# JasperSnoek/spearmint

Measured on AMD Instinct MI355X. Metric: EI candidate evaluations per second (N_cand x mcmc_iters / wall time), higher is better.
Workload: dtype f64; 1 GPU; C3: synthetic 32D, N_obs=2048, 200k candidates/GPU, mcmc_iters=20; N_obs=2048, candidates_per_gpu=200000, D=32, mcmc_iters=20, collective=torch.distributed all_gather_into_tensor

## Files before the change

### spearmint_amd/csrc/common.h

```cpp
#pragma once
#include <hip/hip_runtime.h>
#include <stdint.h>

typedef double d4 __attribute__((ext_vector_type(4)));
typedef double d2 __attribute__((ext_vector_type(2)));

#define MFMA_F64(a, b, c) __builtin_amdgcn_mfma_f64_16x16x4f64((a), (b), (c), 0, 0, 0)

#define SPX_NB 64
#define SPX_BM 128
#define SPX_BN 128
#define SPX_BK 16
#define SPX_PADN 128

#define SPX_COV_MATERN52 0
#define SPX_COV_MATERN32 1
#define SPX_COV_ARDSE 2

#define SPX_HT 4

static inline int64_t round_up(int64_t x, int64_t m) { return (x + m - 1) / m * m; }

void spx_note_attr_error(const char* kernel, size_t lds_bytes, hipError_t e);
#define SPX_LDS_ATTR(fn, bytes)                                                                                            \
// ... 5 lines not shown

void launch_scale_rows(hipStream_t s, const double* x, int64_t n, int64_t n_pad, int D, int Dp,
                       const double* ls , int ls_stride, int nh, double factor,
                       double* xs , double* sumsq ,
                       double* xs2 = nullptr ,
                       int* zero_ints = nullptr , int n_zero = 0);
void launch_lean_prologue(hipStream_t s, const double* x, int64_t n, int64_t n_pad, int D, int Dp, const double* ls,
                          int ls_stride, int nh, double* xs, double* sumsq, double* xs2, const double* vals,
                          const double* htab, double* rhs, int* info, int* flags, int64_t vals_stride = 0);
void launch_cov_self(hipStream_t s, const double* Xs, const double* s1, const double* X2s,
                     const double* htab, double* K, int N, int Np, int Dp, int nh, bool tiled = false,
                     int kind = SPX_COV_MATERN52);
void launch_cov_cross(hipStream_t s, const double* Xs, const double* s1, const double* Cs,
                      const double* s2, const double* htab, double* Kst, int N, int Np, int Mc,
                      int Dp, int nh, int kind = SPX_COV_MATERN52, int live_rows = 0 ,
                      bool allow_flat = true );
void launch_cross_mean(hipStream_t s, const double* Xs, const double* s1, const double* Cs,
                       const double* s2, const double* htab, const double* alpha, double* out,
                       int N, int Np, int Mc, int Dp, int nh, int kind = SPX_COV_MATERN52);
void launch_constraint_prob(hipStream_t s, const double* Xs, const double* s1, const double* Cs,
                            const double* s2, const double* htab, const double* alpha, double* out,
                            int N, int Np, int Mc, int Dp, int nh, int kind);
void launch_constraint_const(hipStream_t s, const double* htab, double* out, int Mc, int nh);

void launch_chol_diag(hipStream_t s, double* L, double* Dinv, int* info, int Np, int k, int nh, int updated = 0);
void launch_chol_panel(hipStream_t s, double* L, const double* Dinv, int Np, int k, int nh, double* rhs = nullptr);
void launch_lean_step(hipStream_t s, double* Lt, double* Dinv, int* info, double* rhs, double* diagL, int Np, int k,
                      int nh, int lazy);
void launch_lean_trsm(hipStream_t s, double* Lt, const double* Dinv, double* rhs, int Np, int k, int nh);
void launch_lean_step_ps(hipStream_t s, double* Lt, double* Dinv, int* info, double* rhs, double* diagL, int* flags,
                         int Np, int k, int nh);
// ... 55 lines not shown
    double* uvec;
};
void launch_point_finish(hipStream_t s, const FinishArgs& a, bool constrained);

void launch_ei_fused128(hipStream_t s, int kind, const double* WT, const double* gamma, const double* Xs, const double* s1,
                        const double* Cs, const double* s2, const double* htab, const double* time_m, const double* cprob, double best,
                        double* ei_draw, double* mom_m, double* mom_v, int N, int Mc, int Dp, int nh, int64_t c0,
                        int64_t M, int64_t Mp, int n_cu);

void launch_sobol_grid(hipStream_t s, const uint32_t* dirs, int dim, int64_t n, int64_t skip, double* out);

void launch_predict_gemm(hipStream_t s, int variant, const double* WT, const double* Kst, const double* gamma,
                         double* part_ss, double* part_bg, int Np, int Mc, int nh, int part_nh, int part_h0,
                         const double* gammaS = nullptr, int S = 0, double* part_bgS = nullptr, int nlive = 0);
bool predict_gemm_variant_ok(int v);
int predict_gemm_padding_plan(int variant, int N, int Np);
void launch_ei_finalize_fant(hipStream_t s, const double* part_ss, const double* part_bgS,
                             const double* htab, const double* bests, const double* time_m, const double* cprob,
                             double* ei_draw, int nrb, int Mc, int nh, int S, int64_t c0, int64_t M,
                             int64_t Mp, int h0, double* ei_s);
void launch_ei_finalize(hipStream_t s, const double* part_ss, const double* part_bg,
                        const double* htab, const double* time_m, const double* cprob, double best, double* ei_draw,
                        double* mom_m, double* mom_v, int nrb, int Mc, int nh, int64_t c0,
                        int64_t M, int64_t Mp, int h0);
void launch_mean_over_draws(hipStream_t s, const double* ei_draw, double* ei_mean, int64_t M,
                            int64_t Mp, int H);
void launch_sum_over_draws(hipStream_t s, const double* ei_draw, double* out, int64_t M, int64_t Mp, int H);
void launch_div_scalar(hipStream_t s, double* v, int64_t n, double denom);
void launch_argmax(hipStream_t s, const double* v, int64_t M, double* blk_val, int64_t* blk_idx,
                   double* out_val, int64_t* out_idx, double* host_mirror = nullptr, const int* info = nullptr, int n_info = 0);
// ... 5 lines not shown
```

### spearmint_amd/csrc/cov_kernels.hip

```cpp
#include "common.h"
#include "ei_device.h"

#ifndef SPX_COV_HOIST
#define SPX_COV_HOIST 1
#endif

#define SR_DC 32
template <int ROWS>
__device__ __forceinline__ void scale_rows_body(
    const double* __restrict__ x, int64_t n, int64_t n_pad, int D, int Dp,
    const double* __restrict__ ls, int ls_stride, double factor,
    double* __restrict__ xs, double* __restrict__ sumsq, double* __restrict__ xs2, int bx, int h)
{
#pragma clang fp contract(off)
    __shared__ double T[ROWS][SR_DC + 1];
    const int tid = threadIdx.x;
    const int64_t row0 = (int64_t)bx * ROWS;
    const int rows = (int)((n_pad - row0 < ROWS) ? (n_pad - row0) : ROWS);
    const int64_t row = row0 + tid;
    const double* lsh = ls + (size_t)h * ls_stride;
    double* o = xs + ((size_t)h * n_pad + row0) * Dp;
    double* o2 = xs2 ? xs2 + ((size_t)h * n_pad + row0) * Dp : nullptr;
    double acc = 0.0;
    for (int d0 = 0; d0 < Dp; d0 += SR_DC) {
// ... 242 lines not shown

template <int MODE, int QC, int KIND>
__global__ __launch_bounds__(256, 2) void k_cov(
    const double* __restrict__ Xs, const double* __restrict__ s1,
    const double* __restrict__ Cs, const double* __restrict__ s2,
    const double* __restrict__ htab, const double* __restrict__ alpha,
    double* __restrict__ out, int N, int Np, int Mc, int Dp, int nchunks, int64_t ldo, int rows_per_wg, int live_rows)
{
    const int jtop = (MODE == 0 && live_rows > 0) ? live_rows : Np;
    const int jbeg = (MODE == 2 || MODE == 4) ? 0 : blockIdx.y * rows_per_wg;
    const int jend = (MODE == 2 || MODE == 4) ? Np : min(jtop, jbeg + rows_per_wg);
    cov_run<MODE, QC, KIND>(Xs, s1, Cs, s2, htab, alpha, out, N, Np, Mc, Dp, nchunks, ldo, blockIdx.z, blockIdx.x * 64, jbeg, jend);
}

template <int QC, int KIND>
__global__ __launch_bounds__(256, 2) void k_cov_flat(
    const double* __restrict__ Xs, const double* __restrict__ s1,
    const double* __restrict__ Cs, const double* __restrict__ s2,
    const double* __restrict__ htab, double* __restrict__ out, int N, int Np, int Mc, int Dp, int nchunks, int64_t ldo, int nh,
    int live_rows)
{
    const int jtop = live_rows > 0 ? live_rows : Np;
    const int nrc = (jtop + 127) >> 7, ncb = Mc >> 6;
    const int64_t per_h = (int64_t)ncb * nrc, U = per_h * nh;
    int64_t u = U * blockIdx.x / gridDim.x;
    const int64_t u1 = U * (blockIdx.x + 1) / gridDim.x;
    while (u < u1) {
        const int h = (int)(u / per_h);
        const int rem = (int)(u - (int64_t)h * per_h);
        const int cb = rem / nrc, rc = rem - cb * nrc;
        const int run = (int)min((int64_t)(nrc - rc), u1 - u);
        cov_run<0, QC, KIND>(Xs, s1, Cs, s2, htab, nullptr, out, N, Np, Mc, Dp, nchunks, ldo, h, cb * 64, rc * 128,
                             min(jtop, (rc + run) * 128));
        u += run;
    }
}

template <int MODE, int KIND>
static void launch_cov_kind(hipStream_t s, const double* Xs, const double* s1, const double* Cs,
                            const double* s2, const double* htab, const double* alpha, double* out,
                            int N, int Np, int Mc, int Dp, int nh, int64_t ldo, int live_rows, bool allow_flat)
{
    const int Q = Dp / 4;
    int rows_per_wg = (Np >= 1024) ? 512 : ((Np >= 256) ? 256 : 128);
#ifdef SPX_DEV_KNOBS
    static const char* rpw = getenv("SPX_COV_RPW");
    if (rpw && MODE == 3) rows_per_wg = atoi(rpw);
#endif
    const int row_top = (MODE == 0 && live_rows > 0) ? live_rows : Np;
    dim3 grid(Mc / 64, (MODE == 2 || MODE == 4) ? 1 : (row_top + rows_per_wg - 1) / rows_per_wg, nh);
// ... 25 lines not shown
}

template <int MODE>
static void launch_cov_mode(hipStream_t s, int kind, const double* Xs, const double* s1, const double* Cs,
                            const double* s2, const double* htab, const double* alpha, double* out,
                            int N, int Np, int Mc, int Dp, int nh, int64_t ldo, int live_rows = 0, bool allow_flat = true)
{
    if (kind == SPX_COV_MATERN32)
        launch_cov_kind<MODE, SPX_COV_MATERN32>(s, Xs, s1, Cs, s2, htab, alpha, out, N, Np, Mc, Dp, nh, ldo, live_rows, allow_flat);
    else if (kind == SPX_COV_ARDSE)
        launch_cov_kind<MODE, SPX_COV_ARDSE>(s, Xs, s1, Cs, s2, htab, alpha, out, N, Np, Mc, Dp, nh, ldo, live_rows, allow_flat);
    else
        launch_cov_kind<MODE, SPX_COV_MATERN52>(s, Xs, s1, Cs, s2, htab, alpha, out, N, Np, Mc, Dp, nh, ldo, live_rows, allow_flat);
}

void launch_cov_cross(hipStream_t s, const double* Xs, const double* s1, const double* Cs,
                      const double* s2, const double* htab, double* Kst, int N, int Np, int Mc,
                      int Dp, int nh, int kind, int live_rows, bool allow_flat)
{
    launch_cov_mode<0>(s, kind, Xs, s1, Cs, s2, htab, nullptr, Kst, N, Np, Mc, Dp, nh, Mc, live_rows, allow_flat);
}

void launch_cov_self(hipStream_t s, const double* Xs, const double* s1, const double* X2s,
                     const double* htab, double* K, int N, int Np, int Dp, int nh, bool tiled, int kind)
{
    if (tiled) launch_cov_mode<3>(s, kind, Xs, s1, X2s, s1, htab, nullptr, K, N, Np, Np, Dp, nh, Np);
    else launch_cov_mode<1>(s, kind, Xs, s1, X2s, s1, htab, nullptr, K, N, Np, Np, Dp, nh, Np);
}

void launch_cross_mean(hipStream_t s, const double* Xs, const double* s1, const double* Cs,
                       const double* s2, const double* htab, const double* alpha, double* out,
                       int N, int Np, int Mc, int Dp, int nh, int kind)
{
    launch_cov_mode<2>(s, kind, Xs, s1, Cs, s2, htab, alpha, out, N, Np, Mc, Dp, nh, Mc);
// ... 21 lines not shown
```

### spearmint_amd/csrc/predict_kernels.hip

```cpp
#include "common.h"
#include "np_sum.h"
#include "ei_device.h"

#define BM SPX_BM
#define BN SPX_BN
#define BK SPX_BK
#define LDT 144

template <int NW, int STG, int ABL>
__global__ __launch_bounds__(64 * NW, NW / 2) void k_predict_gemm(
    const double* __restrict__ WT, const double* __restrict__ Kst,
    const double* __restrict__ gamma, double* __restrict__ part_ss,
    double* __restrict__ part_bg, int Np, int Mc, int nh, int ncb, int nrb,
    int part_nh , int part_h0 ,
    const double* __restrict__ gammaS , int S,
    double* __restrict__ part_bgS )
{
    extern __shared__ __attribute__((aligned(16))) double smem[];
    double* As = smem;
    double* Bs = smem + 2 * BK * LDT;

    const int tid = threadIdx.x;
    const int lane = tid & 63, wave = tid >> 6;
    const int g = lane >> 4, li = lane & 15;
// ... 204 lines not shown
#pragma unroll
            for (int nt = 0; nt < 4; ++nt) {
                double bg = 0.0;
#pragma unroll
                for (int mt = 0; mt < MT; ++mt)
#pragma unroll
                    for (int r = 0; r < 4; ++r) bg = fma(acc[mt][nt][r], gv[mt][r], bg);
                bg += __shfl_xor(bg, 16);
                bg += __shfl_xor(bg, 32);
                if (g == 0) outS[(size_t)sidx * Mc + 16 * nt + li] = bg;
            }
        }
    }
}

__global__ __launch_bounds__(256, 2) void k_predict_gemm_tri(
    const double* __restrict__ WT, const double* __restrict__ Kst,
    const double* __restrict__ gamma, double* __restrict__ part_ss,
    double* __restrict__ part_bg, int Np, int Mc, int nh, int ncb, int nrb,
    int part_nh, int part_h0, const double* __restrict__ gammaS, int S, double* __restrict__ part_bgS)
{
    extern __shared__ __attribute__((aligned(16))) double smem[];
    double* As = smem;
    double* Bs = smem + 2 * BK * LDT;
    const int tid = threadIdx.x;
    const int lane = tid & 63;
    const int wave = __builtin_amdgcn_readfirstlane(tid >> 6);
    const int g = lane >> 4, li = lane & 15;
    const int wm = wave >> 1, wn = wave & 1;
    constexpr int NW = 4, NQ = 4;

    const int ncbx = (ncb + 7) >> 3;
    const int xcd = blockIdx.x & 7;
    const int slot = blockIdx.x >> 3;
    const int per_rb = ncbx * nh;
    const int ib = nrb - 1 - slot / per_rb;
// ... 39 lines not shown
        if (m0 == 0) {
#pragma unroll
            for (int k0 = 0; k0 < BK; k0 += 4) {
                double a[4], b[4];
#pragma unroll
                for (int t = 0; t < 4; ++t) b[t] = Bc[(k0 + g) * LDT + 16 * t];
#pragma unroll
                for (int t = 0; t < 4; ++t) a[t] = Ac[(k0 + g) * LDT + 32 * t];
#pragma unroll
                for (int mt = 0; mt < 4; ++mt)
#pragma unroll
                    for (int nt = 0; nt < 4; ++nt) acc[mt][nt] = MFMA_F64(a[mt], b[nt], acc[mt][nt]);
            }
            asm volatile("s_waitcnt vmcnt(0)" ::: "memory");
            __syncthreads();
        } else {
#define SPX_TRI_G4(MT_)                                                      \
    _Pragma("unroll") for (int nt = 0; nt < 4; ++nt) acc[MT_][nt] = MFMA_F64(a[MT_], b[nt], acc[MT_][nt]);
#pragma unroll
            for (int k0 = 0; k0 < BK; k0 += 4) {
                double a[4], b[4];
#pragma unroll
                for (int t = 0; t < 4; ++t) b[t] = Bc[(k0 + g) * LDT + 16 * t];
#pragma unroll
                for (int t = 0; t < 4; ++t) a[t] = Ac[(k0 + g) * LDT + 32 * t];
                switch (m0) {
                    case 1: SPX_TRI_G4(1)
                    case 2: SPX_TRI_G4(2)
                    case 3: SPX_TRI_G4(3)
                    default: break;
                }
            }
#undef SPX_TRI_G4
            asm volatile("s_waitcnt vmcnt(0)" ::: "memory");
            __syncthreads();
        }
        cur ^= 1;
    }
#undef SPX_DMA_TILE
#undef SPX_DMA_ROW

    const double* gh = gamma + (size_t)h * Np + (size_t)ib * BM + 16 * wm;
    double gam[4][4];
#pragma unroll
    for (int mt = 0; mt < 4; ++mt)
#pragma unroll
        for (int r = 0; r < 4; ++r) gam[mt][r] = gh[32 * mt + g + 4 * r];
    double* red = smem;
// ... 44 lines not shown
                bg += __shfl_xor(bg, 16);
                bg += __shfl_xor(bg, 32);
                if (g == 0) outS[(size_t)sidx * Mc + 16 * nt + li] = bg;
            }
        }
    }
}

template <int ML>
__global__ __launch_bounds__(256, 2) void k_predict_gemm_tail(
    const double* __restrict__ WT, const double* __restrict__ Kst,
    const double* __restrict__ gamma, double* __restrict__ part_ss,
    double* __restrict__ part_bg, int Np, int Mc, int nh, int ncb, int ib, int nlive,
    int part_nh, int part_h0, const double* __restrict__ gammaS, int S, double* __restrict__ part_bgS)
{
    extern __shared__ __attribute__((aligned(16))) double smem[];
    double* As = smem;
    double* Bs = smem + 2 * BK * LDT;
    const int tid = threadIdx.x;
    const int lane = tid & 63;
    const int wave = __builtin_amdgcn_readfirstlane(tid >> 6);
    const int g = lane >> 4, li = lane & 15;
    const int wm = wave >> 1, wn = wave & 1;
    constexpr int NW = 4, NQ = 4;

    const int ncbx = (ncb + 7) >> 3;
    const int xcd = blockIdx.x & 7;
    const int slot = blockIdx.x >> 3;
    const int h = slot / ncbx;
    const int cb = (slot % ncbx) * 8 + xcd;
// ... 139 lines not shown
        default: return false;
    }
}

template <int NW, int STG, int ABL>
static void launch_gemm_variant(hipStream_t s, int grid, size_t lds, const double* WT, const double* Kst,
                                const double* gamma, double* part_ss, double* part_bg, int Np, int Mc, int nh,
                                int ncb, int nrb, int part_nh, int part_h0, const double* gammaS, int S,
                                double* part_bgS)
{
    SPX_LDS_ATTR((k_predict_gemm<NW, STG, ABL>), lds);
    hipLaunchKernelGGL((k_predict_gemm<NW, STG, ABL>), dim3(grid), dim3(64 * NW), lds, s, WT, Kst, gamma, part_ss,
                       part_bg, Np, Mc, nh, ncb, nrb, part_nh, part_h0, gammaS, S, part_bgS);
}

void launch_predict_gemm(hipStream_t s, int variant, const double* WT, const double* Kst, const double* gamma,
                         double* part_ss, double* part_bg, int Np, int Mc, int nh, int part_nh, int part_h0,
                         const double* gammaS, int S, double* part_bgS, int nlive)
{
    const int ncb = Mc / BN, nrb = Np / BM;
    const size_t lds = (size_t)(4 * BK * LDT) * sizeof(double);
    const int grid = 8 * ((ncb + 7) / 8) * nrb * nh;
#define SPX_GO(NW_, STG_, ABL_)                                                                               \
    launch_gemm_variant<NW_, STG_, ABL_>(s, grid, lds, WT, Kst, gamma, part_ss, part_bg, Np, Mc, nh, ncb, nrb, \
                                         part_nh, part_h0, gammaS, S, part_bgS)
    const int v = (S > 0 && variant != 0 && variant != 32) ? 14 : variant;
    if (v == 0 || v == 32) {
        const bool tail = nlive > 0 && predict_gemm_padding_plan(v, 16 * nlive, Np) == nlive;
        const int nrb_main = tail ? nrb - 1 : nrb;
        if (tail) {
            const int lt = nlive - 8 * (nrb - 1), ml = (lt + 1) / 2;
            const int tgrid = 8 * ((ncb + 7) / 8) * nh;
#define SPX_TAIL(ML_)                                                                                                   \
    do {                                                                                                                \
        SPX_LDS_ATTR(k_predict_gemm_tail<ML_>, lds);                                                                    \
        hipLaunchKernelGGL(k_predict_gemm_tail<ML_>, dim3(tgrid), dim3(256), lds, s, WT, Kst, gamma, part_ss, part_bg, Np, Mc, \
// ... 272 lines not shown
```

### spearmint_amd/csrc/spx_api.hip

```cpp
#include <math.h>
#include <stdarg.h>
#include <stdio.h>
#include <string.h>

#include <algorithm>
#include <string>
#include <vector>

#include <chrono>

#include "spx_internal.h"
#include "np_sum.h"

#define SPX_VERSION 200

static const char* kStageNames[ST_COUNT] = {
    "scale_rows", "cov_self", "chol_diag", "chol_panel", "trinv", "gamma_alpha",
    "cov_cross", "cross_mean", "predict_gemm", "ei_finalize", "mean_argmax",
    "factor_total", "ei_run_total"};


std::string& spx_err_slot()
{
    static thread_local std::string g_err;
// ... 22 lines not shown
    va_start(ap, fmt);
    vsnprintf(buf, sizeof buf, fmt, ap);
    va_end(ap);
    spx_err_slot() = buf;
    if (!spx_attr_err_slot().empty()) {
        spx_err_slot() += " [also: " + spx_attr_err_slot() + "]";
        spx_attr_err_slot().clear();
    }
    return code;
}

static int ensure_init(spx_handle* h)
{
    HIPCHK(hipSetDevice(h->device));
    if (!h->inited) {
        HIPCHK(hipStreamCreateWithFlags(&h->stream, hipStreamNonBlocking));
        HIPCHK(hipStreamCreateWithFlags(&h->stream2, hipStreamNonBlocking));
        for (int i = 0; i < 6; ++i) HIPCHK(hipEventCreateWithFlags(&h->ev_sync[i], hipEventDisableTiming));
        HIPCHK(hipEventCreate(&h->ev_t0));
        HIPCHK(hipEventCreate(&h->ev_t1));
        HIPCHK(hipEventCreateWithFlags(&h->ev_obs, hipEventDisableTiming));
        HIPCHK(hipEventCreateWithFlags(&h->ev_p0, hipEventDisableTiming));
        HIPCHK(hipEventCreateWithFlags(&h->ev_fac, hipEventDisableTiming));
        int ncu = 0;
        if (hipDeviceGetAttribute(&ncu, hipDeviceAttributeMultiprocessorCount, h->device) == hipSuccess && ncu > 0) h->n_cu = ncu;
        h->inited = true;
    }
    return SPX_OK;
}

static int ev_begin(spx_handle* h, int stage, hipStream_t strm)
{
    if (!h->timing) return -1;
    if (h->ev_used == h->ev_pool.size()) {
        spx_handle::Ev e;
        if (hipEventCreate(&e.a) != hipSuccess || hipEventCreate(&e.b) != hipSuccess) return -1;
        h->ev_pool.push_back(e);
    }
    spx_handle::Ev& e = h->ev_pool[h->ev_used];
    e.stage = stage;
    (void)hipEventRecord(e.a, strm);
    return (int)h->ev_used++;
}
static void ev_end(spx_handle* h, int id, hipStream_t strm)
{
// ... 51 lines not shown
    *out = h;
    return SPX_OK;
}

void spx_destroy(spx_handle* h)
{
    if (!h) return;
    if (h->multi) { spx_multi_destroy(h->multi); delete h; return; }
    spx_comm_release(h);
    if (h->con) { spx_destroy(h->con); h->con = nullptr; }
    if (h->full) { spx_destroy(h->full); h->full = nullptr; }
    if (h->inited) {
        (void)hipSetDevice(h->device);
        (void)hipStreamSynchronize(h->stream);
        (void)hipStreamSynchronize(h->stream2);
        DevBuf* bufs[] = {&h->comp, &h->vals, &h->ldur, &h->cand, &h->hyp, &h->htab, &h->Xs, &h->X2s,
                          &h->s1, &h->Lm, &h->WT, &h->Dinv, &h->gamma, &h->alpha, &h->info, &h->lp,
                          &h->Cs[0], &h->s2[0], &h->Kst[0], &h->part_ss[0], &h->part_bg[0], &h->time_m[0],
                          &h->Cs[1], &h->s2[1], &h->Kst[1], &h->part_ss[1], &h->part_bg[1], &h->time_m[1],
                          &h->fantT, &h->gammaS, &h->bests, &h->part_bgS[0], &h->part_bgS[1],
                          &h->pt_x, &h->pt_k, &h->pt_dk, &h->pt_t, &h->pt_z, &h->pt_out, &h->pt_kt, &h->pt_dkt,
                          &h->ei_draw, &h->ei_mean, &h->mom_m, &h->mom_v, &h->mom_t, &h->am_val, &h->am_idx,
                          &h->am_out_val, &h->am_out_idx, &h->scratch, &h->sobol_dirs, &h->sobol_out, &h->rhs, &h->diagL, &h->ps_flags, &h->flow_flags,
                          &h->alphaS, &h->pt_u, &h->rec_send, &h->rec_recv, &h->rec_out, &h->ei_sum_full,
                          &h->con_tab, &h->con_Cs[0], &h->con_Cs[1], &h->con_s2[0], &h->con_s2[1], &h->con_p[0], &h->con_p[1],
                          &h->mom_c, &h->rhs_rows};
        for (DevBuf* b : bufs) b->release();
        h->pin_up.release();
        h->pin_res.release();
        h->pin_stage.release();
// ... 88 lines not shown
    if (!strcmp(name, "lean_poll")) { h->lean_poll = value < 0 ? -1 : (value != 0); return SPX_OK; }
    if (!strcmp(name, "lean_zc")) { h->lean_zc = value < 0 ? -1 : (value != 0); return SPX_OK; }
    if (!strcmp(name, "stage_copies")) {
        h->stage_copies = value < 0 ? -1 : (value != 0);
        return SPX_OK;
    }
    if (!strcmp(name, "cov_flat")) {
        h->cov_flat = value < 0 ? -1 : (value != 0);
        return SPX_OK;
    }
    if (!strcmp(name, "gemm_partial")) {
        h->gemm_partial = value < 0 ? -1 : (value != 0);
        return SPX_OK;
    }
    if (!strcmp(name, "streams")) {
        h->nstreams = value == 2 ? 2 : 1;
        return SPX_OK;
    }
    if (!strcmp(name, "timing")) {
        h->timing = value != 0;
        memset(h->st_ms, 0, sizeof h->st_ms);
        memset(h->st_n, 0, sizeof h->st_n);
        return SPX_OK;
    }
    return fail(SPX_ERR_ARG, "spx_set_option: unknown option '%s'", name);
}

#define SPX_STAGE_MAX (8u << 20)
static void stage_begin(spx_handle* h) { h->stage_off = 0; }
static int stage_h2d(spx_handle* h, void* dst, const void* src, size_t bytes, hipStream_t s)
{
// ... 515 lines not shown
    h->handoff_timeout = false;
    rc = do_factor(h, false, false, true);
    if (rc) return rc;
    h->S = 0;
    rc = ei_run_impl(h, flags, true);
    if (rc == SPX_ERR_HIP && h->handoff_timeout && h->flow_used) {
        note_flow_timeout(h);
        rc = do_factor(h, false);
        if (!rc) rc = ei_run_impl(h, flags, false);
        if (!rc) warn_flow_fallback(h);
        return rc;
    }
    if (rc) {
        (void)hipStreamSynchronize(h->stream);
        (void)hipStreamSynchronize(h->stream2);
        (void)hipGetLastError();
        if (rc != SPX_ERR_NOT_PD) h->factored = false;
    }
    return rc;
}

static int ei_run_impl(spx_handle* h, int32_t flags, bool factor_pending)
{
    if (!h->factored && !factor_pending) return fail(SPX_ERR_ARG, "spx_ei_run: call spx_factor first");
    if (!h->have_cand) return fail(SPX_ERR_ARG, "spx_ei_run: no candidates set");
    const bool per_sec = (flags & SPX_FLAG_PER_SEC) != 0;
    const bool keep_mom = (flags & SPX_FLAG_KEEP_MOMENTS) != 0;
    const bool time_only = (flags & SPX_FLAG_TIME_ONLY) != 0;
    const bool constrained = (flags & SPX_FLAG_CONSTRAINED) != 0;
    int rc = check_run_flags(h, flags, h->nmodels);
// ... 21 lines not shown
        const int64_t fant_budget = h->fant_budget;
        int64_t cap = fant_budget / ((int64_t)nrb * 2 * S * 8) / SPX_BN * SPX_BN;
        if (cap < SPX_BN) cap = SPX_BN;
        if (Mc > cap) {
            const int64_t nchunks = (Mp + cap - 1) / cap;
            Mc = round_up((Mp + nchunks - 1) / nchunks, SPX_BN);
        }
        int64_t hb = fant_budget / ((int64_t)nrb * 2 * S * 8 * Mc);
        if (hb > 65535 / S) hb = 65535 / S;
        if (hb < 1) hb = 1;
        if (hb < Hb) Hb = (int)hb;
    }

    const bool fused = Np == SPX_PADN && S == 0 && h->ei_fused != 0;
    h->last_fused = fused;
    const int ns = fused ? 1 : h->nstreams;
    for (int b = 0; b < 2; ++b) {
        if ((rc = h->Cs[b].reserve((size_t)H * Mc * Dp * 8))) return rc;
        if ((rc = h->s2[b].reserve((size_t)H * Mc * 8))) return rc;
        if (per_sec && (rc = h->time_m[b].reserve((size_t)H * Mc * 8))) return rc;
        if (constrained && (rc = h->con_p[b].reserve((size_t)H * Mc * 8))) return rc;
        if (constrained && h->con_n > 0 && (rc = h->con_Cs[b].reserve((size_t)H * Mc * Dp * 8))) return rc;
        if (constrained && h->con_n > 0 && (rc = h->con_s2[b].reserve((size_t)H * Mc * 8))) return rc;
        if (b < ns && !fused && !time_only) {
            if ((rc = h->Kst[b].reserve((size_t)Hb * Np * Mc * 8))) return rc;
            if (S > 0 && (rc = h->part_bgS[b].reserve((size_t)nrb * 2 * Hb * S * Mc * 8))) return rc;
        }
    }
    if (!fused && !time_only && (rc = h->part_ss[0].reserve((size_t)nrb * H * Mc * 8))) return rc;
    if (!fused && !time_only && (rc = h->part_bg[0].reserve((size_t)nrb * H * Mc * 8))) return rc;
    if (S > 0 && (rc = h->scratch.reserve((size_t)Hb * S * Mc * 8))) return rc;
    if ((rc = h->ei_draw.reserve((size_t)H * Mp * 8))) return rc;
    if ((rc = h->ei_mean.reserve((size_t)Mp * 8))) return rc;
    if (keep_mom) {
        if ((rc = h->mom_m.reserve((size_t)H * Mp * 8))) return rc;
        if ((rc = h->mom_v.reserve((size_t)H * Mp * 8))) return rc;
        if (per_sec && (rc = h->mom_t.reserve((size_t)H * Mp * 8))) return rc;
        if (constrained && (rc = h->mom_c.reserve((size_t)H * Mp * 8))) return rc;
    }
// ... 3 lines not shown
    if ((rc = h->am_out_val.reserve(8))) return rc;
    if ((rc = h->am_out_idx.reserve(8))) return rc;

    hipStream_t s = h->stream;
    if (flags & SPX_FLAG_TIMING) h->timing = true;
    h->ev_used = 0;
    hipEvent_t t0 = h->ev_t0, t1 = h->ev_t1;
    HIPCHK(hipEventRecord(t0, s));
    const int gemm_nlive = (!fused && h->gemm_partial != 0) ? predict_gemm_padding_plan(h->gemm_variant, (int)N, Np) : 0;
    const bool skip_pad = gemm_nlive > 0;
    const int cov_live_rows = 16 * gemm_nlive;
    h->last_skip_pad = skip_pad;

    const double* ls = h->hyp.d() + 3;
    const size_t nn = (size_t)Np * Np;
    hipStream_t G = h->stream, P = (ns == 2) ? h->stream2 : h->stream;
    const bool overlap = factor_pending && ns == 1 && h->step_overlap != 0;
    hipStream_t P0 = overlap ? h->stream2 : P;
    if (overlap) HIPCHK(hipStreamWaitEvent(P0, h->ev_obs, 0));
    if (factor_pending && ns == 2) HIPCHK(hipStreamWaitEvent(P, per_sec ? h->ev_fac : h->ev_obs, 0));
    int item = 0, chunk = 0;
    for (int64_t c0 = 0; c0 < Mp; c0 += Mc, ++chunk) {
        const int mc = (int)std::min<int64_t>(Mc, Mp - c0);
        const int64_t nreal = std::min<int64_t>(mc, M - c0);
        const double* xc = h->cand.d() + (size_t)c0 * D;
        const int par = chunk & 1;
        double* Cs = h->Cs[par].d();
        double* s2 = h->s2[par].d();
        double* tm = per_sec ? h->time_m[par].d() : nullptr;
        if (ns == 2 && chunk >= 2) HIPCHK(hipStreamWaitEvent(P, h->ev_sync[4 + par], 0));
        if (per_sec) {
            const bool side = overlap && chunk == 0;
            hipStream_t T = side ? G : P;
            double* CsT = side ? h->Cs[par ^ 1].d() : Cs;
            double* s2T = side ? h->s2[par ^ 1].d() : s2;
            TIMED_S(ST_SCALE, T, launch_scale_rows(T, xc, nreal, mc, D, Dp, ls + (size_t)H * hs, hs, H, 2.0, CsT, s2T));
            TIMED_S(ST_CROSS_MEAN, T, launch_cross_mean(T, h->Xs.d() + (size_t)H * Np * Dp, h->s1.d() + (size_t)H * Np, CsT, s2T,
                                                        h->htab.d() + (size_t)H * SPX_HT, h->alpha.d() + (size_t)H * Np, tm,
                                                        (int)N, Np, mc, Dp, H, dev_kind(h)));
            if (keep_mom)
                HIPCHK(hipMemcpy2DAsync(h->mom_t.d() + c0, (size_t)Mp * 8, tm, (size_t)mc * 8,
                                        (size_t)std::min<int64_t>(mc, Mp - c0) * 8, (size_t)H, hipMemcpyDeviceToDevice, T));
        }
        if (time_only) continue;
        double* cp = constrained ? h->con_p[par].d() : nullptr;
// ... 12 lines not shown
                HIPCHK(hipMemcpy2DAsync(h->mom_c.d() + c0, (size_t)Mp * 8, cp, (size_t)mc * 8,
                                        (size_t)std::min<int64_t>(mc, Mp - c0) * 8, (size_t)H, hipMemcpyDeviceToDevice, P));
        }
        hipStream_t Pc = (chunk == 0) ? P0 : P;
        TIMED_S(ST_SCALE, Pc, launch_scale_rows(Pc, xc, nreal, mc, D, Dp, ls, hs, H, 2.0, Cs, s2));
        if (fused && Pc != G) {
            HIPCHK(hipEventRecord(h->ev_p0, Pc));
            HIPCHK(hipStreamWaitEvent(G, h->ev_p0, 0));
        }
        if (fused)
            TIMED_S(ST_PREDICT_GEMM, G, launch_ei_fused128(G, dev_kind(h), h->WT.d(), h->gamma.d(), h->Xs.d(), h->s1.d(), Cs, s2,
                                                           h->htab.d(), tm, cp, h->best, h->ei_draw.d(), keep_mom ? h->mom_m.d() : nullptr,
                                                           keep_mom ? h->mom_v.d() : nullptr, (int)N, mc, Dp, H, c0, M, Mp, h->n_cu));
        for (int h0 = 0; h0 < (fused ? 0 : H); h0 += Hb, ++item) {
            const int nhb = std::min(Hb, H - h0);
            const int k = (ns == 2) ? (item & 1) : 0;
            if (ns == 2 && item >= 2) HIPCHK(hipStreamWaitEvent(P, h->ev_sync[2 + k], 0));
            hipStream_t Pi = (item == 0) ? Pc : P;
            TIMED_S(ST_COV_CROSS, Pi, launch_cov_cross(Pi, h->Xs.d() + (size_t)h0 * Np * Dp, h->s1.d() + (size_t)h0 * Np,
                                                      Cs + (size_t)h0 * mc * Dp, s2 + (size_t)h0 * mc,
                                                      h->htab.d() + (size_t)h0 * SPX_HT, h->Kst[k].d(), (int)N, Np, mc, Dp, nhb, dev_kind(h),
                                                      cov_live_rows, h->cov_flat != 0));
            if (ns == 2) {
                HIPCHK(hipEventRecord(h->ev_sync[k], P));
                HIPCHK(hipStreamWaitEvent(G, h->ev_sync[k], 0));
            } else if (Pi != G) {
                HIPCHK(hipEventRecord(h->ev_p0, Pi));
                HIPCHK(hipStreamWaitEvent(G, h->ev_p0, 0));
            }
            TIMED_S(ST_PREDICT_GEMM, G, launch_predict_gemm(G, h->gemm_variant, h->WT.d() + (size_t)h0 * nn, h->Kst[k].d(),
                                                            h->gamma.d() + (size_t)h0 * Np, h->part_ss[0].d(),
                                                            h->part_bg[0].d(), Np, mc, nhb, S > 0 ? nhb : H, S > 0 ? 0 : h0,
                                                            S > 0 ? h->gammaS.d() + (size_t)h0 * S * Np : nullptr, S,
                                                            S > 0 ? h->part_bgS[k].d() : nullptr, gemm_nlive));
            if (S > 0)
                TIMED_S(ST_EI_FINALIZE, G, launch_ei_finalize_fant(G, h->part_ss[0].d(), h->part_bgS[k].d(),
                                                                   h->htab.d() + (size_t)h0 * SPX_HT,
                                                                   h->bests.d() + (size_t)h0 * S,
                                                                   per_sec ? tm + (size_t)h0 * mc : nullptr,
                                                                   constrained ? cp + (size_t)h0 * mc : nullptr,
                                                                   h->ei_draw.d(), nrb, mc, nhb, S, c0, M, Mp, h0,
                                                                   h->scratch.d()));
            if (ns == 2) HIPCHK(hipEventRecord(h->ev_sync[2 + k], G));
        }
        if (S == 0 && !fused)
            TIMED_S(ST_EI_FINALIZE, G, launch_ei_finalize(G, h->part_ss[0].d(), h->part_bg[0].d(), h->htab.d(), tm, cp, h->best,
                                                          h->ei_draw.d(), keep_mom ? h->mom_m.d() : nullptr,
                                                          keep_mom ? h->mom_v.d() : nullptr, nrb, mc, H, c0, M, Mp, 0));
        if (ns == 2) HIPCHK(hipEventRecord(h->ev_sync[4 + par], G));
    }
    if (ns == 2 && (per_sec || constrained) && keep_mom) {
        HIPCHK(hipEventRecord(h->ev_sync[0], P));
        HIPCHK(hipStreamWaitEvent(G, h->ev_sync[0], 0));
    }
    const int n_info = factor_pending ? h->nmodels * H : 0;
    if ((rc = h->pin_res.reserve(16 + (size_t)n_info * sizeof(int)))) return rc;
    double* mirror = (double*)h->pin_res.p;
    TIMED(ST_MEAN_ARGMAX, {
        launch_mean_argmax(s, h->ei_draw.d(), h->ei_mean.d(), M, Mp, H, h->am_val.d(), (int64_t*)h->am_idx.p, h->am_out_val.d(),
                           (int64_t*)h->am_out_idx.p, mirror, (const int*)h->info.p, n_info);
    });
    HIPCHK(hipEventRecord(t1, s));
    HIPCHK(hipStreamSynchronize(s));
    LAUNCHCHK();
    h->best_val = mirror[0];
    h->best_idx = ((const int64_t*)mirror)[1];
// ... 560 lines not shown
{
    if (!h || !name || !value) return fail(SPX_ERR_ARG, "spx_get_stat: null");
    if (h->multi) {
        if (!strcmp(name, "ranks_seen") || !strcmp(name, "flow_fallbacks") || !strcmp(name, "flow_rearms") || !strcmp(name, "obs_dims"))
            return spx_multi_stat(h->multi, name, value);
        return fail(SPX_ERR_ARG, "spx_get_stat: ask the per-device handles (single-GPU handles only)");
    }
    if (!strcmp(name, "flow_fallbacks")) *value = h->flow_fallbacks;
    else if (!strcmp(name, "flow_enabled")) *value = (h->lean_flow != 0 && !h->flow_demoted);
    else if (!strcmp(name, "flow_rearms")) *value = h->flow_rearms;
    else if (!strcmp(name, "ranks_seen")) *value = h->comm ? h->ranks_seen : 1;
    else if (!strcmp(name, "n_cu")) *value = h->n_cu;
    else if (!strcmp(name, "obs_dims")) *value = h->have_obs ? h->D : 0;
    else if (!strcmp(name, "last_step_fused")) *value = h->last_fused ? 1 : 0;
    else if (!strcmp(name, "last_step_skipped_padding")) *value = h->last_skip_pad ? 1 : 0;
    else if (!strcmp(name, "hip_runtime_version") || !strcmp(name, "hip_driver_version")) {
        int v = 0;
        HIPCHK(name[4] == 'r' ? hipRuntimeGetVersion(&v) : hipDriverGetVersion(&v));
        *value = v;
    } else if (!strcmp(name, "clock_khz") || !strcmp(name, "mem_clock_khz") || !strcmp(name, "wall_clock_khz")
               || !strcmp(name, "l2_bytes") || !strcmp(name, "mem_bus_bits")) {
        int rc = ensure_init(h);
        if (rc) return rc;
        int v = 0;
        const hipDeviceAttribute_t a = !strcmp(name, "clock_khz") ? hipDeviceAttributeClockRate
            : !strcmp(name, "mem_clock_khz") ? hipDeviceAttributeMemoryClockRate
            : !strcmp(name, "wall_clock_khz") ? hipDeviceAttributeWallClockRate
            : !strcmp(name, "l2_bytes") ? hipDeviceAttributeL2CacheSize : hipDeviceAttributeMemoryBusWidth;
        HIPCHK(hipDeviceGetAttribute(&v, a, h->device));
        *value = v;
// ... 20 lines not shown
```

### spearmint_amd/csrc/spx_internal.h

```cpp
#pragma once
#include <stdarg.h>
#include <stdio.h>
#include <string.h>

#include <string>
#include <vector>

#include "../../include/spx.h"
#include "common.h"

std::string& spx_err_slot();
int spx_fail(int code, const char* fmt, ...);
#define fail spx_fail

#define HIPCHK(call)                                                                          \
    do {                                                                                      \
        hipError_t e_ = (call);                                                               \
        if (e_ != hipSuccess) {                                                               \
            (void)hipGetLastError();    \
            return fail(SPX_ERR_HIP, "%s failed: %s (%s:%d)", #call, hipGetErrorString(e_),   \
                        __FILE__, __LINE__);                                                  \
        }                                                                                     \
    } while (0)

// ... 40 lines not shown
        if (bytes <= cap) return SPX_OK;
        if (p) { (void)hipHostFree(p); p = nullptr; cap = 0; }
        if (bytes < 4096) bytes = 4096;
        hipError_t e = hipHostMalloc(&p, bytes, hipHostMallocCoherent);
        if (e != hipSuccess) {
            p = nullptr;
            (void)hipGetLastError();
            return fail(SPX_ERR_HIP, "hipHostMalloc(%zu bytes) failed: %s", bytes, hipGetErrorString(e));
        }
        cap = bytes;
        return SPX_OK;
    }
    void release() { if (p) (void)hipHostFree(p); p = nullptr; cap = 0; }
};

enum Stage {
    ST_SCALE = 0, ST_COV_SELF, ST_CHOL_DIAG, ST_CHOL_PANEL, ST_TRINV, ST_GAMMA_ALPHA,
    ST_COV_CROSS, ST_CROSS_MEAN, ST_PREDICT_GEMM, ST_EI_FINALIZE, ST_MEAN_ARGMAX,
    ST_FACTOR_TOTAL, ST_EI_RUN_TOTAL, ST_COUNT
};
struct spx_handle {
    int device = 0;
    bool inited = false;
    hipStream_t stream = nullptr;
    hipStream_t stream2 = nullptr;
    hipEvent_t ev_sync[6] = {nullptr, nullptr, nullptr, nullptr, nullptr, nullptr};
    hipEvent_t ev_t0 = nullptr, ev_t1 = nullptr;
    hipEvent_t ev_fac = nullptr;
    hipEvent_t ev_obs = nullptr, ev_p0 = nullptr;

    int64_t N = 0, M = 0, index_base = 0;
    int D = 0, Dp = 0, Np = 0, H = 0;
    bool have_obs = false, have_cand = false, have_hyp = false, have_time = false;
    bool factored = false, ran = false, ran_moments = false;
    bool ran_time = false;
    bool ran_tmean = false;
    int nmodels = 1;
    double best = 0.0;
    int not_pd_draw = -1, not_pd_pivot = -1;
    int64_t kst_budget = 512ll << 20;
    int nstreams = 1;
// ... 124 lines not shown
```

Baseline: 15.16 million EI evals/s.

## Add ring-buffered three-stream K* pipeline with co-run cov kernel and GEMM priority

Adds a third low-priority stream and a ring of K* buffers, so cross-covariance tiles for many items can be produced ahead of the predict GEMM on a high-priority main stream. A co-run cov kernel variant with capped VGPRs and a sized grid is meant to share CUs with the GEMM. The GEMM kernels raise their wave priority via s_setprio, and the triangular GEMM inner loop is restructured. This costs extra device memory for the ring and adds event bookkeeping. The ring path only runs when streams=3 is selected.

After: 15.39 million EI evals/s (median of 6 runs). 1.5% higher.

```diff
diff --git a/spearmint_amd/csrc/common.h b/spearmint_amd/csrc/common.h
--- a/spearmint_amd/csrc/common.h
+++ b/spearmint_amd/csrc/common.h
@@ -43,7 +43,8 @@
 void launch_cov_cross(hipStream_t s, const double* Xs, const double* s1, const double* Cs,
                       const double* s2, const double* htab, double* Kst, int N, int Np, int Mc,
                       int Dp, int nh, int kind = SPX_COV_MATERN52, int live_rows = 0 ,
-                      bool allow_flat = true );
+                      bool allow_flat = true ,
+                      bool corun = false );
 void launch_cross_mean(hipStream_t s, const double* Xs, const double* s1, const double* Cs,
                        const double* s2, const double* htab, const double* alpha, double* out,
                        int N, int Np, int Mc, int Dp, int nh, int kind = SPX_COV_MATERN52);
@@ -129,6 +130,7 @@
                          double* part_ss, double* part_bg, int Np, int Mc, int nh, int part_nh, int part_h0,
                          const double* gammaS = nullptr, int S = 0, double* part_bgS = nullptr, int nlive = 0);
 bool predict_gemm_variant_ok(int v);
+size_t predict_gemm_lds_bytes();
 int predict_gemm_padding_plan(int variant, int N, int Np);
 void launch_ei_finalize_fant(hipStream_t s, const double* part_ss, const double* part_bgS,
                              const double* htab, const double* bests, const double* time_m, const double* cprob,
diff --git a/spearmint_amd/csrc/cov_kernels.hip b/spearmint_amd/csrc/cov_kernels.hip
--- a/spearmint_amd/csrc/cov_kernels.hip
+++ b/spearmint_amd/csrc/cov_kernels.hip
@@ -280,17 +280,17 @@
 }
 
 template <int QC, int KIND>
-__global__ __launch_bounds__(256, 2) void k_cov_flat(
+__device__ __forceinline__ void cov_flat_share(
     const double* __restrict__ Xs, const double* __restrict__ s1,
     const double* __restrict__ Cs, const double* __restrict__ s2,
     const double* __restrict__ htab, double* __restrict__ out, int N, int Np, int Mc, int Dp, int nchunks, int64_t ldo, int nh,
-    int live_rows)
+    int live_rows, unsigned blk, unsigned nblk)
 {
     const int jtop = live_rows > 0 ? live_rows : Np;
     const int nrc = (jtop + 127) >> 7, ncb = Mc >> 6;
     const int64_t per_h = (int64_t)ncb * nrc, U = per_h * nh;
-    int64_t u = U * blockIdx.x / gridDim.x;
-    const int64_t u1 = U * (blockIdx.x + 1) / gridDim.x;
+    int64_t u = U * blk / nblk;
+    const int64_t u1 = U * (blk + 1) / nblk;
     while (u < u1) {
         const int h = (int)(u / per_h);
         const int rem = (int)(u - (int64_t)h * per_h);
@@ -300,6 +300,27 @@
                              min(jtop, (rc + run) * 128));
         u += run;
     }
+}
+
+template <int QC, int KIND>
+__global__ __launch_bounds__(256, 2) void k_cov_flat(
+    const double* __restrict__ Xs, const double* __restrict__ s1,
+    const double* __restrict__ Cs, const double* __restrict__ s2,
+    const double* __restrict__ htab, double* __restrict__ out, int N, int Np, int Mc, int Dp, int nchunks, int64_t ldo, int nh,
+    int live_rows)
+{
+    cov_flat_share<QC, KIND>(Xs, s1, Cs, s2, htab, out, N, Np, Mc, Dp, nchunks, ldo, nh, live_rows, blockIdx.x, gridDim.x);
+}
+
+template <int QC, int KIND>
+__global__ __launch_bounds__(256, 2) __attribute__((amdgpu_num_vgpr(152))) void k_cov_corun(
+    const double* __restrict__ Xs, const double* __restrict__ s1,
+    const double* __restrict__ Cs, const double* __restrict__ s2,
+    const double* __restrict__ htab, double* __restrict__ out, int N, int Np, int Mc, int Dp, int nchunks, int64_t ldo, int nh,
+    int live_rows)
+{
+    static_assert(QC <= 4, "the co-run form keeps at most four column-side quads in registers");
+    cov_flat_share<QC, KIND>(Xs, s1, Cs, s2, htab, out, N, Np, Mc, Dp, nchunks, ldo, nh, live_rows, blockIdx.x, gridDim.x);
 }
 
 template <int MODE, int KIND>
@@ -355,10 +376,37 @@
         launch_cov_kind<MODE, SPX_COV_MATERN52>(s, Xs, s1, Cs, s2, htab, alpha, out, N, Np, Mc, Dp, nh, ldo, live_rows, allow_flat);
 }
 
+template <int KIND>
+static void launch_cov_corun_kind(hipStream_t s, const double* Xs, const double* s1, const double* Cs, const double* s2,
+                                  const double* htab, double* out, int N, int Np, int Mc, int Dp, int nh, int64_t ldo,
+                                  int live_rows)
+{
+    const int Q = Dp / 4;
+    const int64_t places = spx_cov_cus();
+    const int64_t units = (int64_t)nh * (Mc / 64) * (((live_rows > 0 ? live_rows : Np) + 127) / 128);
+    const int64_t rounds = (units + 16 * places - 1) / (16 * places);
+    const dim3 grid((unsigned)(places * rounds));
+#define SPX_COVC_LAUNCH(QC_)                                                                                   \
+    hipLaunchKernelGGL((k_cov_corun<QC_, KIND>), grid, dim3(256), 0, s, Xs, s1, Cs, s2, htab, out, N, Np, Mc, Dp, Q / QC_, ldo, nh, live_rows)
+    if (Q == 1) SPX_COVC_LAUNCH(1);
+    else if (Q == 2) SPX_COVC_LAUNCH(2);
+    else SPX_COVC_LAUNCH(4);
+#undef SPX_COVC_LAUNCH
+}
+
 void launch_cov_cross(hipStream_t s, const double* Xs, const double* s1, const double* Cs,
                       const double* s2, const double* htab, double* Kst, int N, int Np, int Mc,
-                      int Dp, int nh, int kind, int live_rows, bool allow_flat)
-{
+                      int Dp, int nh, int kind, int live_rows, bool allow_flat, bool corun)
+{
+    if (corun && allow_flat) {
+        if (kind == SPX_COV_MATERN32)
+            launch_cov_corun_kind<SPX_COV_MATERN32>(s, Xs, s1, Cs, s2, htab, Kst, N, Np, Mc, Dp, nh, Mc, live_rows);
+        else if (kind == SPX_COV_ARDSE)
+            launch_cov_corun_kind<SPX_COV_ARDSE>(s, Xs, s1, Cs, s2, htab, Kst, N, Np, Mc, Dp, nh, Mc, live_rows);
+        else
+            launch_cov_corun_kind<SPX_COV_MATERN52>(s, Xs, s1, Cs, s2, htab, Kst, N, Np, Mc, Dp, nh, Mc, live_rows);
+        return;
+    }
     launch_cov_mode<0>(s, kind, Xs, s1, Cs, s2, htab, nullptr, Kst, N, Np, Mc, Dp, nh, Mc, live_rows, allow_flat);
 }
 
diff --git a/spearmint_amd/csrc/predict_kernels.hip b/spearmint_amd/csrc/predict_kernels.hip
--- a/spearmint_amd/csrc/predict_kernels.hip
+++ b/spearmint_amd/csrc/predict_kernels.hip
@@ -242,12 +242,21 @@
     }
 }
 
+#ifndef SPX_GEMM_PRIO
+#define SPX_GEMM_PRIO 3
+#endif
+#define SPX_GEMM_SETPRIO()                                                \
+    do {                                                                  \
+        if (SPX_GEMM_PRIO > 0) __builtin_amdgcn_s_setprio(SPX_GEMM_PRIO); \
+    } while (0)
+
 __global__ __launch_bounds__(256, 2) void k_predict_gemm_tri(
     const double* __restrict__ WT, const double* __restrict__ Kst,
     const double* __restrict__ gamma, double* __restrict__ part_ss,
     double* __restrict__ part_bg, int Np, int Mc, int nh, int ncb, int nrb,
     int part_nh, int part_h0, const double* __restrict__ gammaS, int S, double* __restrict__ part_bgS)
 {
+    SPX_GEMM_SETPRIO();
     extern __shared__ __attribute__((aligned(16))) double smem[];
     double* As = smem;
     double* Bs = smem + 2 * BK * LDT;
@@ -317,24 +326,23 @@
             }
             asm volatile("s_waitcnt vmcnt(0)" ::: "memory");
             __syncthreads();
-        } else {
-#define SPX_TRI_G4(MT_)                                                      \
-    _Pragma("unroll") for (int nt = 0; nt < 4; ++nt) acc[MT_][nt] = MFMA_F64(a[MT_], b[nt], acc[MT_][nt]);
+        }
+        int md = m0;
+        asm volatile("" : "+s"(md));
+        if (md != 0) {
 #pragma unroll
             for (int k0 = 0; k0 < BK; k0 += 4) {
-                double a[4], b[4];
+                double b[4];
 #pragma unroll
                 for (int t = 0; t < 4; ++t) b[t] = Bc[(k0 + g) * LDT + 16 * t];
 #pragma unroll
-                for (int t = 0; t < 4; ++t) a[t] = Ac[(k0 + g) * LDT + 32 * t];
-                switch (m0) {
-                    case 1: SPX_TRI_G4(1)
-                    case 2: SPX_TRI_G4(2)
-                    case 3: SPX_TRI_G4(3)
-                    default: break;
-                }
-            }
-#undef SPX_TRI_G4
+                for (int mt = 1; mt < 4; ++mt)
+                    if (mt >= m0) {
+                        const double a = Ac[(k0 + g) * LDT + 32 * mt];
+#pragma unroll
+                        for (int nt = 0; nt < 4; ++nt) acc[mt][nt] = MFMA_F64(a, b[nt], acc[mt][nt]);
+                    }
+            }
             asm volatile("s_waitcnt vmcnt(0)" ::: "memory");
             __syncthreads();
         }
@@ -409,6 +417,7 @@
     double* __restrict__ part_bg, int Np, int Mc, int nh, int ncb, int ib, int nlive,
     int part_nh, int part_h0, const double* __restrict__ gammaS, int S, double* __restrict__ part_bgS)
 {
+    SPX_GEMM_SETPRIO();
     extern __shared__ __attribute__((aligned(16))) double smem[];
     double* As = smem;
     double* Bs = smem + 2 * BK * LDT;
@@ -578,12 +587,14 @@
                        part_bg, Np, Mc, nh, ncb, nrb, part_nh, part_h0, gammaS, S, part_bgS);
 }
 
+size_t predict_gemm_lds_bytes() { return (size_t)(4 * BK * LDT) * sizeof(double); }
+
 void launch_predict_gemm(hipStream_t s, int variant, const double* WT, const double* Kst, const double* gamma,
                          double* part_ss, double* part_bg, int Np, int Mc, int nh, int part_nh, int part_h0,
                          const double* gammaS, int S, double* part_bgS, int nlive)
 {
     const int ncb = Mc / BN, nrb = Np / BM;
-    const size_t lds = (size_t)(4 * BK * LDT) * sizeof(double);
+    const size_t lds = predict_gemm_lds_bytes();
     const int grid = 8 * ((ncb + 7) / 8) * nrb * nh;
 #define SPX_GO(NW_, STG_, ABL_)                                                                               \
     launch_gemm_variant<NW_, STG_, ABL_>(s, grid, lds, WT, Kst, gamma, part_ss, part_bg, Np, Mc, nh, ncb, nrb, \
diff --git a/spearmint_amd/csrc/spx_api.hip b/spearmint_amd/csrc/spx_api.hip
--- a/spearmint_amd/csrc/spx_api.hip
+++ b/spearmint_amd/csrc/spx_api.hip
@@ -60,7 +60,9 @@
 {
     HIPCHK(hipSetDevice(h->device));
     if (!h->inited) {
-        HIPCHK(hipStreamCreateWithFlags(&h->stream, hipStreamNonBlocking));
+        int prio_least = 0, prio_greatest = 0;
+        if (hipDeviceGetStreamPriorityRange(&prio_least, &prio_greatest) != hipSuccess) { (void)hipGetLastError(); prio_least = prio_greatest = 0; }
+        HIPCHK(hipStreamCreateWithPriority(&h->stream, hipStreamNonBlocking, prio_greatest));
         HIPCHK(hipStreamCreateWithFlags(&h->stream2, hipStreamNonBlocking));
         for (int i = 0; i < 6; ++i) HIPCHK(hipEventCreateWithFlags(&h->ev_sync[i], hipEventDisableTiming));
         HIPCHK(hipEventCreate(&h->ev_t0));
@@ -75,6 +77,31 @@
     return SPX_OK;
 }
 
+static int ensure_ring(spx_handle* h, int R)
+{
+    if (!h->stream3) {
+        int prio_least = 0, prio_greatest = 0;
+        if (hipDeviceGetStreamPriorityRange(&prio_least, &prio_greatest) != hipSuccess) { (void)hipGetLastError(); prio_least = prio_greatest = 0; }
+        HIPCHK(hipStreamCreateWithPriority(&h->stream3, hipStreamNonBlocking, prio_least));
+    }
+    while ((int)h->ring.size() < R) {
+        spx_handle::RingSlot sl;
+        HIPCHK(hipEventCreateWithFlags(&sl.ready, hipEventDisableTiming));
+        hipError_t e = hipEventCreateWithFlags(&sl.consumed, hipEventDisableTiming);
+        if (e != hipSuccess) {
+            (void)hipEventDestroy(sl.ready);
+            (void)hipGetLastError();
+            return fail(SPX_ERR_HIP, "hipEventCreateWithFlags failed: %s", hipGetErrorString(e));
+        }
+        h->ring.push_back(sl);
+    }
+    return SPX_OK;
+}
+static void ring_trim(spx_handle* h, int keep)
+{
+    for (size_t i = (size_t)std::max(keep, 0); i < h->ring.size(); ++i) { h->ring[i].Kst.release(); h->ring[i].part_bgS.release(); }
+}
+
 static int ev_begin(spx_handle* h, int stage, hipStream_t strm)
 {
     if (!h->timing) return -1;
@@ -156,6 +183,15 @@
         (void)hipSetDevice(h->device);
         (void)hipStreamSynchronize(h->stream);
         (void)hipStreamSynchronize(h->stream2);
+        if (h->stream3) (void)hipStreamSynchronize(h->stream3);
+        for (auto& sl : h->ring) {
+            sl.Kst.release();
+            sl.part_bgS.release();
+            (void)hipEventDestroy(sl.ready);
+            (void)hipEventDestroy(sl.consumed);
+        }
+        h->ring.clear();
+        if (h->stream3) (void)hipStreamDestroy(h->stream3);
         DevBuf* bufs[] = {&h->comp, &h->vals, &h->ldur, &h->cand, &h->hyp, &h->htab, &h->Xs, &h->X2s,
                           &h->s1, &h->Lm, &h->WT, &h->Dinv, &h->gamma, &h->alpha, &h->info, &h->lp,
                           &h->Cs[0], &h->s2[0], &h->Kst[0], &h->part_ss[0], &h->part_bg[0], &h->time_m[0],
@@ -274,7 +310,15 @@
         return SPX_OK;
     }
     if (!strcmp(name, "streams")) {
-        h->nstreams = value == 2 ? 2 : 1;
+        h->nstreams = (value == 2 || value == 3) ? (int)value : 1;
+        return SPX_OK;
+    }
+    if (!strcmp(name, "kstar_ring")) {
+        h->ring_opt = value <= 0 ? 0 : (int)std::min<int64_t>(value, 4096);
+        return SPX_OK;
+    }
+    if (!strcmp(name, "kstar_corun")) {
+        h->corun_opt = value < 0 ? -1 : (value != 0);
         return SPX_OK;
     }
     if (!strcmp(name, "timing")) {
@@ -820,6 +864,7 @@
     if (rc) {
         (void)hipStreamSynchronize(h->stream);
         (void)hipStreamSynchronize(h->stream2);
+        if (h->stream3) (void)hipStreamSynchronize(h->stream3);
         (void)hipGetLastError();
         if (rc != SPX_ERR_NOT_PD) h->factored = false;
     }
@@ -871,7 +916,37 @@
 
     const bool fused = Np == SPX_PADN && S == 0 && h->ei_fused != 0;
     h->last_fused = fused;
-    const int ns = fused ? 1 : h->nstreams;
+    const bool timing_on = h->timing || (flags & SPX_FLAG_TIMING);
+    const int ns = fused ? 1 : ((h->nstreams == 3 && timing_on) ? 1 : h->nstreams);
+    const bool ringed = ns == 3 && !time_only;
+    int R = 0;
+    if (ringed) {
+        const int64_t slot = (int64_t)Hb * Np * Mc * 8 + (S > 0 ? (int64_t)nrb * 2 * Hb * S * Mc * 8 : 0);
+        if (h->ring_budget_slot != slot) {
+            size_t mem_free = 0, mem_total = 0;
+            int64_t b = 10ll << 30;
+            if (hipMemGetInfo(&mem_free, &mem_total) == hipSuccess) {
+                int64_t held = 0;
+                for (auto& sl : h->ring) held += (int64_t)(sl.Kst.cap + sl.part_bgS.cap);
+                b = std::min<int64_t>(b, (int64_t)(mem_free / 16) + held);
+            } else (void)hipGetLastError();
+            h->ring_budget = b;
+            h->ring_budget_slot = slot;
+        }
+        const int64_t nitems = ((Mp + Mc - 1) / Mc) * ((H + Hb - 1) / Hb);
+        int64_t r = h->ring_opt > 0 ? h->ring_opt : h->ring_budget / slot;
+        r = std::max<int64_t>(1, std::min<int64_t>(std::min<int64_t>(r, nitems), 4096));
+        R = (int)r;
+        if ((rc = ensure_ring(h, R))) return rc;
+        for (int k = 0; k < R; ++k) {
+            if ((rc = h->ring[k].Kst.reserve((size_t)Hb * Np * Mc * 8))) return rc;
+            if (S > 0 && (rc = h->ring[k].part_bgS.reserve((size_t)nrb * 2 * Hb * S * Mc * 8))) return rc;
+        }
+    }
+    if (ns == 3 && !ringed && (rc = ensure_ring(h, 0))) return rc;
+    if (ringed || h->nstreams != 3) ring_trim(h, R);
+    h->ring_used = R;
+    h->corun_launches = 0;
     for (int b = 0; b < 2; ++b) {
         if ((rc = h->Cs[b].reserve((size_t)H * Mc * Dp * 8))) return rc;
         if ((rc = h->s2[b].reserve((size_t)H * Mc * 8))) return rc;
@@ -879,7 +954,7 @@
         if (constrained && (rc = h->con_p[b].reserve((size_t)H * Mc * 8))) return rc;
         if (constrained && h->con_n > 0 && (rc = h->con_Cs[b].reserve((size_t)H * Mc * Dp * 8))) return rc;
         if (constrained && h->con_n > 0 && (rc = h->con_s2[b].reserve((size_t)H * Mc * 8))) return rc;
-        if (b < ns && !fused && !time_only) {
+        if (b < ns && ns <= 2 && !fused && !time_only) {
             if ((rc = h->Kst[b].reserve((size_t)Hb * Np * Mc * 8))) return rc;
             if (S > 0 && (rc = h->part_bgS[b].reserve((size_t)nrb * 2 * Hb * S * Mc * 8))) return rc;
         }
@@ -913,11 +988,12 @@
 
     const double* ls = h->hyp.d() + 3;
     const size_t nn = (size_t)Np * Np;
-    hipStream_t G = h->stream, P = (ns == 2) ? h->stream2 : h->stream;
+    hipStream_t G = h->stream, P = (ns == 3) ? h->stream3 : (ns == 2) ? h->stream2 : h->stream;
+    const int64_t ring_items = ringed ? ((Mp + Mc - 1) / Mc) * ((H + Hb - 1) / Hb) : 0;
     const bool overlap = factor_pending && ns == 1 && h->step_overlap != 0;
     hipStream_t P0 = overlap ? h->stream2 : P;
     if (overlap) HIPCHK(hipStreamWaitEvent(P0, h->ev_obs, 0));
-    if (factor_pending && ns == 2) HIPCHK(hipStreamWaitEvent(P, per_sec ? h->ev_fac : h->ev_obs, 0));
+    if (factor_pending && ns >= 2) HIPCHK(hipStreamWaitEvent(P, per_sec ? h->ev_fac : h->ev_obs, 0));
     int item = 0, chunk = 0;
     for (int64_t c0 = 0; c0 < Mp; c0 += Mc, ++chunk) {
         const int mc = (int)std::min<int64_t>(Mc, Mp - c0);
@@ -927,7 +1003,7 @@
         double* Cs = h->Cs[par].d();
         double* s2 = h->s2[par].d();
         double* tm = per_sec ? h->time_m[par].d() : nullptr;
-        if (ns == 2 && chunk >= 2) HIPCHK(hipStreamWaitEvent(P, h->ev_sync[4 + par], 0));
+        if (ns >= 2 && chunk >= 2) HIPCHK(hipStreamWaitEvent(P, h->ev_sync[4 + par], 0));
         if (per_sec) {
             const bool side = overlap && chunk == 0;
             hipStream_t T = side ? G : P;
@@ -970,27 +1046,35 @@
                                                            keep_mom ? h->mom_v.d() : nullptr, (int)N, mc, Dp, H, c0, M, Mp, h->n_cu));
         for (int h0 = 0; h0 < (fused ? 0 : H); h0 += Hb, ++item) {
             const int nhb = std::min(Hb, H - h0);
-            const int k = (ns == 2) ? (item & 1) : 0;
+            const int k = (ns == 3) ? item % R : (ns == 2) ? (item & 1) : 0;
             if (ns == 2 && item >= 2) HIPCHK(hipStreamWaitEvent(P, h->ev_sync[2 + k], 0));
+            if (ns == 3 && item >= R) HIPCHK(hipStreamWaitEvent(P, h->ring[k].consumed, 0));
             hipStream_t Pi = (item == 0) ? Pc : P;
+            double* Kst_k = (ns == 3) ? h->ring[k].Kst.d() : h->Kst[k].d();
+            double* bgS_k = S > 0 ? ((ns == 3) ? h->ring[k].part_bgS.d() : h->part_bgS[k].d()) : nullptr;
+            const bool corun = ns == 3 && item > 0 && h->corun_opt != 0 && h->cov_flat != 0;
+            h->corun_launches += corun ? 1 : 0;
             TIMED_S(ST_COV_CROSS, Pi, launch_cov_cross(Pi, h->Xs.d() + (size_t)h0 * Np * Dp, h->s1.d() + (size_t)h0 * Np,
                                                       Cs + (size_t)h0 * mc * Dp, s2 + (size_t)h0 * mc,
-                                                      h->htab.d() + (size_t)h0 * SPX_HT, h->Kst[k].d(), (int)N, Np, mc, Dp, nhb, dev_kind(h),
-                                                      cov_live_rows, h->cov_flat != 0));
-            if (ns == 2) {
+                                                      h->htab.d() + (size_t)h0 * SPX_HT, Kst_k, (int)N, Np, mc, Dp, nhb, dev_kind(h),
+                                                      cov_live_rows, h->cov_flat != 0, corun));
+            if (ns == 3) {
+                HIPCHK(hipEventRecord(h->ring[k].ready, P));
+                HIPCHK(hipStreamWaitEvent(G, h->ring[k].ready, 0));
+            } else if (ns == 2) {
                 HIPCHK(hipEventRecord(h->ev_sync[k], P));
                 HIPCHK(hipStreamWaitEvent(G, h->ev_sync[k], 0));
             } else if (Pi != G) {
                 HIPCHK(hipEventRecord(h->ev_p0, Pi));
                 HIPCHK(hipStreamWaitEvent(G, h->ev_p0, 0));
             }
-            TIMED_S(ST_PREDICT_GEMM, G, launch_predict_gemm(G, h->gemm_variant, h->WT.d() + (size_t)h0 * nn, h->Kst[k].d(),
+            TIMED_S(ST_PREDICT_GEMM, G, launch_predict_gemm(G, h->gemm_variant, h->WT.d() + (size_t)h0 * nn, Kst_k,
                                                             h->gamma.d() + (size_t)h0 * Np, h->part_ss[0].d(),
                                                             h->part_bg[0].d(), Np, mc, nhb, S > 0 ? nhb : H, S > 0 ? 0 : h0,
                                                             S > 0 ? h->gammaS.d() + (size_t)h0 * S * Np : nullptr, S,
-                                                            S > 0 ? h->part_bgS[k].d() : nullptr, gemm_nlive));
+                                                            bgS_k, gemm_nlive));
             if (S > 0)
-                TIMED_S(ST_EI_FINALIZE, G, launch_ei_finalize_fant(G, h->part_ss[0].d(), h->part_bgS[k].d(),
+                TIMED_S(ST_EI_FINALIZE, G, launch_ei_finalize_fant(G, h->part_ss[0].d(), bgS_k,
                                                                    h->htab.d() + (size_t)h0 * SPX_HT,
                                                                    h->bests.d() + (size_t)h0 * S,
                                                                    per_sec ? tm + (size_t)h0 * mc : nullptr,
@@ -998,14 +1082,15 @@
                                                                    h->ei_draw.d(), nrb, mc, nhb, S, c0, M, Mp, h0,
                                                                    h->scratch.d()));
             if (ns == 2) HIPCHK(hipEventRecord(h->ev_sync[2 + k], G));
+            if (ns == 3 && (int64_t)item + R < ring_items) HIPCHK(hipEventRecord(h->ring[k].consumed, G));
         }
         if (S == 0 && !fused)
             TIMED_S(ST_EI_FINALIZE, G, launch_ei_finalize(G, h->part_ss[0].d(), h->part_bg[0].d(), h->htab.d(), tm, cp, h->best,
                                                           h->ei_draw.d(), keep_mom ? h->mom_m.d() : nullptr,
                                                           keep_mom ? h->mom_v.d() : nullptr, nrb, mc, H, c0, M, Mp, 0));
-        if (ns == 2) HIPCHK(hipEventRecord(h->ev_sync[4 + par], G));
-    }
-    if (ns == 2 && (per_sec || constrained) && keep_mom) {
+        if (ns >= 2) HIPCHK(hipEventRecord(h->ev_sync[4 + par], G));
+    }
+    if (ns >= 2 && (per_sec || constrained) && keep_mom) {
         HIPCHK(hipEventRecord(h->ev_sync[0], P));
         HIPCHK(hipStreamWaitEvent(G, h->ev_sync[0], 0));
     }
@@ -1596,6 +1681,9 @@
     else if (!strcmp(name, "obs_dims")) *value = h->have_obs ? h->D : 0;
     else if (!strcmp(name, "last_step_fused")) *value = h->last_fused ? 1 : 0;
     else if (!strcmp(name, "last_step_skipped_padding")) *value = h->last_skip_pad ? 1 : 0;
+    else if (!strcmp(name, "last_corun_launches")) *value = h->corun_launches;
+    else if (!strcmp(name, "last_kstar_ring")) *value = h->ring_used;
+    else if (!strcmp(name, "gemm_lds_bytes")) *value = (int64_t)predict_gemm_lds_bytes();
     else if (!strcmp(name, "hip_runtime_version") || !strcmp(name, "hip_driver_version")) {
         int v = 0;
         HIPCHK(name[4] == 'r' ? hipRuntimeGetVersion(&v) : hipDriverGetVersion(&v));
diff --git a/spearmint_amd/csrc/spx_internal.h b/spearmint_amd/csrc/spx_internal.h
--- a/spearmint_amd/csrc/spx_internal.h
+++ b/spearmint_amd/csrc/spx_internal.h
@@ -78,6 +78,10 @@
     void release() { if (p) (void)hipHostFree(p); p = nullptr; cap = 0; }
 };
 
+#ifndef SPX_DEFAULT_CORUN
+#define SPX_DEFAULT_CORUN -1
+#endif
+
 enum Stage {
     ST_SCALE = 0, ST_COV_SELF, ST_CHOL_DIAG, ST_CHOL_PANEL, ST_TRINV, ST_GAMMA_ALPHA,
     ST_COV_CROSS, ST_CROSS_MEAN, ST_PREDICT_GEMM, ST_EI_FINALIZE, ST_MEAN_ARGMAX,
@@ -89,6 +93,15 @@
     hipStream_t stream = nullptr;
     hipStream_t stream2 = nullptr;
     hipEvent_t ev_sync[6] = {nullptr, nullptr, nullptr, nullptr, nullptr, nullptr};
+    hipStream_t stream3 = nullptr;
+    struct RingSlot { DevBuf Kst, part_bgS; hipEvent_t ready = nullptr, consumed = nullptr; };
+    std::vector<RingSlot> ring;
+    int ring_opt = 0;
+    int corun_opt = SPX_DEFAULT_CORUN;
+    int64_t ring_budget = 0;
+    int64_t ring_budget_slot = -1;
+    int ring_used = 0;
+    int corun_launches = 0;
     hipEvent_t ev_t0 = nullptr, ev_t1 = nullptr;
     hipEvent_t ev_fac = nullptr;
     hipEvent_t ev_obs = nullptr, ev_p0 = nullptr;
```
